# stardist/stardist

Measured on AMD Instinct MI355X. Metric: predict_instances() Mpix/s (2D) + Mvox/s (3D) end-to-end at 1/2/4/8 GPU, higher is better.
Workload: dtype f32

## Files before the change

### stardist_amd/csrc/clip_beam.h

```cpp
#pragma once
#include "clip_sweep.h"
#include <limits.h>

#if defined(BEAM_COUNT) && !defined(__HIP_DEVICE_COMPILE__)
struct BeamCounters { long beams, topx, isect_pt, isect_edges, outpt, update, maxima, lm, horz, ael_sum, il_beams, es_loads; };
inline BeamCounters& beam_counters() { static BeamCounters c = {}; return c; }
#define BEAM_CNT(f, v) (beam_counters().f += (v))
#else
#define BEAM_CNT(f, v) ((void)0)
#endif

namespace sdclip {

typedef unsigned long long u64;

enum {
  ST_OVERFLOW_AEL = 32,
  ST_OVERFLOW_LM = 64,
  ST_OVERFLOW_GJ = 128
};
enum { BEAM_MAXLM = 8 };

struct PrepPt { int x, y; };
template <bool WIDE> struct PrepIdx { typedef unsigned char type; enum { NONE = 255 }; };
template <> struct PrepIdx<true> { typedef unsigned short type; enum { NONE = 65535 }; };
template <int MAXV>
struct PolyPrep {
  typedef typename PrepIdx<(MAXV > 128)>::type pidx;
  enum { NONE = PrepIdx<(MAXV > 128)>::NONE };
  int n;
  int n_lm;
  int status;
  int pad;
  PrepPt v[MAXV + 1];
  unsigned char ecode[MAXV];
  pidx mpair[MAXV];
  pidx hlast[MAXV];
  pidx lm_left[BEAM_MAXLM], lm_right[BEAM_MAXLM];
};

#ifndef BEAM_PREP_IDX
#define BEAM_PREP_IDX short
#endif
// ... 183 lines not shown
      else if (topx(b) == topx(i) && topy(b) == topy(i) && (code[b] & 3) == 0) mp = b;
      out->mpair[i] = (typename PolyPrep<MAXV>::pidx)mp;
      int last = i, g2 = 0;
      if (is_horz(i)) {
        for (;;) {
          const int c2 = code[last] & 3;
          const int n2 = (c2 == 1) ? nx(last) : (c2 == 2 ? pv(last) : -1);
          if (n2 < 0 || !is_horz(n2)) break;
          last = n2;
          if (++g2 > MAXV) { st |= ST_ITER; break; }
        }
      }
      out->hlast[i] = (typename PolyPrep<MAXV>::pidx)last;
    }
    for (int i = 0; i < n_lm; ++i) { out->lm_left[i] = (typename PolyPrep<MAXV>::pidx)lml_[i]; out->lm_right[i] = (typename PolyPrep<MAXV>::pidx)lmr_[i]; }
    out->n = m; out->n_lm = n_lm; out->status = st;
  }
};

template <class D, class P, int MAXV, int K, int MAXIL, bool FULLGJ = false>
struct BeamCore {
  typedef PolyPrep<MAXV> Prep;
  template <bool W, int = 0> struct OrdT { typedef unsigned int type; };
  template <int D0> struct OrdT<true, D0> { typedef u64 type; };
  typedef typename OrdT<(K > 8)>::type ord_t;
  enum { ORD_BITS = (K > 8) ? 64 : 32 };
  enum { GJ = (K <= 8 ? 3 : 4), NX = (K <= 8 ? 2 : 4), EID_POLY = 4096 };
  SD_HD D& self() { return *static_cast<D*>(this); }
  static constexpr unsigned RI = P::template coord_region<K>(), RD = P::template slope_region<K>(),
                            RS = P::template region<short, K>(), RB = P::template region<signed char, K>(),
                            RIL = P::template coord_region<MAXIL>(), RILB = P::template region<signed char, MAXIL>(),
                            RG = P::template coord_region<GJ>(), RGF = P::template region<int, (FULLGJ ? GJ : 1)>(), R1 = P::template region<int, 1>(), R8 = P::template region<u64, 1>(), RO = P::template region<ord_t, 1>();
  static constexpr unsigned O_BOTX = 0, O_BOTY = O_BOTX + RI, O_TOPX = O_BOTY + RI, O_TOPY = O_TOPX + RI, O_CURX = O_TOPY + RI,
                            O_CURY = O_CURX + RI, O_DX = O_CURY + RI, O_EID = O_DX + RD, O_WCNT = O_EID + RS, O_WCNT2 = O_WCNT + RB,
                            O_OUTIDX = O_WCNT2 + RB, O_LMLC = O_OUTIDX + RB, O_WDELTA = O_LMLC + RB, O_PTYP = O_WDELTA + RB,
                            O_SIDE = O_PTYP + RB, O_ILX = O_SIDE + RB, O_ILY = O_ILX + RIL, O_ILE1 = O_ILY + RIL, O_ILE2 = O_ILE1 + RILB,
                            O_GJOP = O_ILE2 + RILB, O_GJX1 = O_GJOP + RGF, O_GJX2 = O_GJX1 + RG, O_GJY2 = O_GJX2 + RG,
                            O_XTRA = O_GJY2 + RGF, O_MLM = O_XTRA + P::template region<int, NX>(),
                            O_PA = O_MLM + P::template region<unsigned char, 16>(),
                            O_ORD = O_PA + 2 * R8, O_HSEL = O_ORD + RO, O_AFTER_ORD = O_HSEL + RO, O_PB = O_PA + R8, O_NAEL = O_AFTER_ORD, O_FREE = O_NAEL + R1, O_NLM = O_FREE + R1,
                            O_CURLM = O_NLM + R1, O_NIL = O_CURLM + R1, O_STATUS = O_NIL + R1, O_NJOINS = O_STATUS + R1,
                            O_NGJ = O_NJOINS + R1, O_NXTRA = O_NGJ + R1, O_LMY = O_NXTRA + R1, O_ORGX = O_LMY + R1, O_ORGY = O_ORGX + R1, O_CORE_END = O_ORGY + R1;
  typename P::template CoordArr<K, O_BOTX, O_ORGX, O_STATUS> botx; typename P::template CoordArr<K, O_BOTY, O_ORGY, O_STATUS> boty;
  typename P::template CoordArr<K, O_TOPX, O_ORGX, O_STATUS> topx; typename P::template CoordArr<K, O_TOPY, O_ORGY, O_STATUS> topy;
  typename P::template CoordArr<K, O_CURX, O_ORGX, O_STATUS> curx; typename P::template CoordArr<K, O_CURY, O_ORGY, O_STATUS> cury;
  typename P::template SlopeArr<K, O_DX, O_BOTX, O_BOTY, O_TOPX, O_TOPY> dx;
  typename P::template Arr<short, K, O_EID> eid;
  typename P::template Arr<signed char, K, O_WCNT> wcnt; typename P::template Arr<signed char, K, O_WCNT2> wcnt2;
  typename P::template Arr<signed char, K, O_OUTIDX> outidx;
  typename P::template Arr<signed char, K, O_LMLC> lmlc;
  typename P::template Arr<signed char, K, O_WDELTA> wdelta; typename P::template Arr<signed char, K, O_PTYP> ptyp;
  typename P::template Arr<signed char, K, O_SIDE> side;
  typename P::template CoordArr<MAXIL, O_ILX, O_ORGX, O_STATUS> ilx; typename P::template CoordArr<MAXIL, O_ILY, O_ORGY, O_STATUS> ily;
  typename P::template Arr<signed char, MAXIL, O_ILE1> ile1; typename P::template Arr<signed char, MAXIL, O_ILE2> ile2;
  typename P::template Arr<int, (FULLGJ ? GJ : 1), O_GJOP> gjop; typename P::template CoordArr<GJ, O_GJX1, O_ORGX, O_STATUS> gjx1;
  typename P::template CoordArr<GJ, O_GJX2, O_ORGX, O_STATUS> gjx2; typename P::template Arr<int, (FULLGJ ? GJ : 1), O_GJY2> gjy2;
  typename P::template Arr<int, NX, O_XTRA> xtra;
  typename P::template Arr<unsigned char, 16, O_MLM> mlm;
  typename P::template Scalar<ord_t, O_ORD> ord;
  typename P::template Scalar<ord_t, O_HSEL> hsel;
  typename P::template Scalar<const Prep*, O_PA> prepA; typename P::template Scalar<const Prep*, O_PB> prepB;
  typename P::template Scalar<int, O_NAEL> n_ael; typename P::template Scalar<int, O_FREE> freemask;
  typename P::template Scalar<int, O_NLM> n_lm; typename P::template Scalar<int, O_CURLM> cur_lm;
  typename P::template Scalar<int, O_NIL> n_il; typename P::template Scalar<int, O_STATUS> status;
  typename P::template Scalar<int, O_NJOINS> n_joins; typename P::template Scalar<int, O_NGJ> n_gj;
  typename P::template Scalar<int, O_NXTRA> n_xtra;
  typename P::template Scalar<int, O_LMY> next_lm_y;
  typename P::template Scalar<int, O_ORGX> orgx; typename P::template Scalar<int, O_ORGY> orgy;

  static constexpr ord_t ALLF = (ord_t)~(ord_t)0;
  static constexpr ord_t ONES = (ord_t)0x1111111111111111ull, HIGHS = (ord_t)0x8888888888888888ull;
  static SD_HD int nib(ord_t w, int p) { return (int)((w >> (4 * p)) & (ord_t)15); }
  static SD_HD int nib_find(ord_t w, int h) {
    const ord_t x = w ^ ((ord_t)h * ONES);
    const ord_t t = (ord_t)(x - ONES) & ~x & HIGHS;
    if (!t) return -1;
#if defined(__HIP_DEVICE_COMPILE__)
    return (ORD_BITS == 64) ? ((__ffsll((long long)t) - 1) >> 2) : ((__ffs((int)t) - 1) >> 2);
#else
    return (ORD_BITS == 64) ? (__builtin_ctzll((u64)t) >> 2) : (__builtin_ctz((unsigned)t) >> 2);
#endif
  }
  static SD_HD ord_t nib_insert(ord_t w, int p, int h) {
    const ord_t lowmask = (p == 0) ? (ord_t)0 : (ord_t)(ALLF >> (ORD_BITS - 4 * p));
    return (ord_t)((w & lowmask) | ((ord_t)h << (4 * p)) | ((ord_t)(w & ~lowmask) << 4));
  }
  static SD_HD ord_t nib_remove(ord_t w, int p) {
    const ord_t lowmask = (p == 0) ? (ord_t)0 : (ord_t)(ALLF >> (ORD_BITS - 4 * p));
    return (ord_t)((w & lowmask) | (((w >> 4) & ~lowmask)) | ((ord_t)0xF << (ORD_BITS - 4)));
  }
  static SD_HD ord_t nib_swap(ord_t w, int p, int q) {
    const ord_t d = (ord_t)(nib(w, p) ^ nib(w, q));
    return (ord_t)(w ^ (d << (4 * p)) ^ (d << (4 * q)));
  }
  SD_HD int ael_head() const { return n_ael > 0 ? nib(ord, 0) : -1; }
  SD_HD int anext(int h) const { const ord_t w = ord; const int p = nib_find(w, h); if (p < 0 || p + 1 >= n_ael) return -1; return nib(w, p + 1); }
  SD_HD int aprev(int h) const { const ord_t w = ord; const int p = nib_find(w, h); if (p <= 0) return -1; return nib(w, p - 1); }
  SD_HD bool in_ael(int h) const { return nib_find(ord, h) >= 0; }
  SD_HD int alloc_slot() {
    const int f = freemask;
    if (!f) { status |= ST_OVERFLOW_AEL; return 0; }
#if defined(__HIP_DEVICE_COMPILE__)
    const int h = __ffs(f) - 1;
#else
    const int h = __builtin_ctz((unsigned)f);
#endif
    freemask = f & (f - 1);
    return h;
  }

  SD_HD const Prep* prep_of(int id) const { return (id >= EID_POLY) ? (const Prep*)prepB : (const Prep*)prepA; }
  static SD_HD int ring_nx(const Prep* q, int i) { return i + 1 == q->n ? 0 : i + 1; }
  static SD_HD int ring_pv(const Prep* q, int i) { return i == 0 ? q->n - 1 : i - 1; }
  struct ES { int bx, by, tx, ty, code; };
  static SD_HD ES edge_static(const Prep* q, int i) {
    BEAM_CNT(es_loads, 1);
    ES s;
    s.code = q->ecode[i];
    const PrepPt p0 = q->v[i], p1 = q->v[i + 1];
    const int x0 = p0.x, y0 = p0.y, x1 = p1.x, y1 = p1.y;
    if (s.code & 4) { s.bx = x1; s.by = y1; s.tx = x0; s.ty = y0; }
    else { s.bx = x0; s.by = y0; s.tx = x1; s.ty = y1; }
    return s;
  }
  SD_HD int lml_id(int id, int code) const {
    const int c = code & 3;
    if (!c) return -1;
    const Prep* q = prep_of(id);
    const int base = id & ~(EID_POLY - 1), i = id & (EID_POLY - 1);
    return base + (c == 1 ? ring_nx(q, i) : ring_pv(q, i));
  }
  SD_HD ES es_of(int id) const { return edge_static(prep_of(id), id & (EID_POLY - 1)); }
  static SD_HD double es_dx(const ES& s) {
    const i64 dy = (i64)s.ty - s.by;
    if (dy == 0) return SD_HORIZONTAL;
    return (double)((i64)s.tx - s.bx) / (double)dy;
  }
  SD_HD void load_slot(int h, int id) {
    const ES s = es_of(id);
    botx[h] = s.bx; boty[h] = s.by; topx[h] = s.tx; topy[h] = s.ty;
    dx[h] = es_dx(s);
    eid[h] = (short)id; lmlc[h] = (signed char)(s.code & 11);
  }

  SD_HD bool is_horz(int h) const { return topy[h] == boty[h]; }
  SD_HD i64 top_x(int h, i64 y) const {
    BEAM_CNT(topx, 1);
    return (y == topy[h]) ? (i64)topx[h] : (i64)botx[h] + sd_round(dx[h] * (double)(y - boty[h]));
  }
  static SD_HD bool slopes_equal4(i64 x1, i64 y1, i64 x2, i64 y2, i64 x3, i64 y3, i64 x4, i64 y4) {
    return (y1 - y2) * (x3 - x4) == (x1 - x2) * (y3 - y4);
  }
  SD_HD bool slopes_equal_e(int e1, int e2) const {
    return ((i64)topy[e1] - boty[e1]) * ((i64)topx[e2] - botx[e2]) ==
           ((i64)topx[e1] - botx[e1]) * ((i64)topy[e2] - boty[e2]);
  }
  static SD_HD bool horz_segments_overlap(i64 a1, i64 a2, i64 b1, i64 b2) {
    if (a1 > a2) { i64 t = a1; a1 = a2; a2 = t; }
    if (b1 > b2) { i64 t = b1; b1 = b2; b2 = t; }
    return (a1 < b2) && (b1 < a2);
  }
  SD_HD void add_join(int op1, int op2, int offx, int offy) { ++n_joins; self().out_add_join(op1, op2, offx, offy); }
  SD_HD void add_ghost_join(int op, int x1, int x2, int y2) {
// ... 92 lines not shown
    int at;
    if (n == 0) at = 0;
    else if (startEdge < 0 && e2_inserts_before_e1(nib(w, 0), edge)) at = 0;
    else {
      int p = (startEdge < 0) ? 0 : nib_find(w, startEdge);
      if (p < 0) p = 0;
      while (p + 1 < n && !e2_inserts_before_e1(nib(w, p + 1), edge)) ++p;
      at = p + 1;
    }
    ord = nib_insert(w, at, edge);
    n_ael = n + 1;
  }
  SD_HD void delete_from_ael(int e) {
    const ord_t w = ord;
    const int p = nib_find(w, e);
    if (p < 0) return;
    ord = nib_remove(w, p);
    n_ael = n_ael - 1;
    freemask = freemask | (1 << e);
  }
  SD_HD void swap_positions_in_ael(int e1, int e2) {
    const ord_t w = ord;
    const int p = nib_find(w, e1), q = nib_find(w, e2);
    if (p < 0 || q < 0) return;
    ord = nib_swap(w, p, q);
  }
  SD_HD void add_edge_to_sel(int edge) { hsel = (ord_t)(((ord_t)hsel << 4) | (ord_t)edge); }
  SD_HDN int update_edge_into_ael(int e) {
    BEAM_CNT(update, 1);
    const int id = eid[e];
    const int n = lml_id(id, lmlc[e]);
    if (n < 0) { status |= ST_FAIL; return e; }
    load_slot(e, n);
    curx[e] = botx[e]; cury[e] = boty[e];
    return e;
  }

  SD_HDN void set_winding_count(int edge) {
    const ord_t w = ord;
    const int pe = nib_find(w, edge);
    int p = pe - 1;
    while (p >= 0 && (ptyp[nib(w, p)] != ptyp[edge] || wdelta[nib(w, p)] == 0)) --p;
    if (p < 0) {
      wcnt[edge] = wdelta[edge];
      wcnt2[edge] = 0;
      p = 0;
    } else {
      const int e = nib(w, p);
      if (wcnt[e] * wdelta[e] < 0) {
        int a = wcnt[e] < 0 ? -wcnt[e] : wcnt[e];
        if (a > 1) {
          if (wdelta[e] * wdelta[edge] < 0) wcnt[edge] = wcnt[e];
          else wcnt[edge] = (signed char)(wcnt[e] + wdelta[edge]);
        } else wcnt[edge] = (wdelta[edge] == 0 ? 1 : wdelta[edge]);
      } else {
        if (wdelta[edge] == 0) wcnt[edge] = (signed char)(wcnt[e] < 0 ? wcnt[e] - 1 : wcnt[e] + 1);
        else if (wdelta[e] * wdelta[edge] < 0) wcnt[edge] = wcnt[e];
        else wcnt[edge] = (signed char)(wcnt[e] + wdelta[edge]);
      }
      wcnt2[edge] = wcnt2[e];
      ++p;
    }
    for (; p < pe; ++p) wcnt2[edge] = (signed char)(wcnt2[edge] + wdelta[nib(w, p)]);
  }
  SD_HD bool is_contributing(int e) const {
    int a = wcnt[e] < 0 ? -wcnt[e] : wcnt[e];
    if (a != 1) return false;
// ... 27 lines not shown
        signed char s = side[e1]; side[e1] = side[e2]; side[e2] = s;
        signed char o = outidx[e1]; outidx[e1] = outidx[e2]; outidx[e2] = o;
      }
    } else if (c2) {
      if (e1Wc == 0 || e1Wc == 1) {
        add_out_pt_t<true>(e2, px, py);
        signed char s = side[e1]; side[e1] = side[e2]; side[e2] = s;
        signed char o = outidx[e1]; outidx[e1] = outidx[e2]; outidx[e2] = o;
      }
    } else if ((e1Wc == 0 || e1Wc == 1) && (e2Wc == 0 || e2Wc == 1)) {
      int e1Wc2 = wcnt2[e1] < 0 ? -wcnt2[e1] : wcnt2[e1];
      int e2Wc2 = wcnt2[e2] < 0 ? -wcnt2[e2] : wcnt2[e2];
      if (ptyp[e1] != ptyp[e2]) add_local_min_poly_t<true>(e1, e2, px, py);
      else if (e1Wc == 1 && e2Wc == 1) {
        if (e1Wc2 > 0 && e2Wc2 > 0) add_local_min_poly_t<true>(e1, e2, px, py);
      } else { signed char s = side[e1]; side[e1] = side[e2]; side[e2] = s; }
    }
  }

  SD_BLK void insert_local_minima_into_ael(int botY) {
    while (cur_lm < n_lm && next_lm_y == botY) {
      const int m = mlm[cur_lm];
      ++cur_lm;
      if (cur_lm < n_lm) next_lm_y = lm_y(cur_lm);
      BEAM_CNT(lm, 1);
      const int poly = (m & 128) ? 1 : 0;
      const Prep* q = poly ? (const Prep*)prepB : (const Prep*)prepA;
      const int li = q->lm_left[m & 127], ri = q->lm_right[m & 127];
      const int lb = alloc_slot();
      const int rb = alloc_slot();
      if (status & ST_OVERFLOW_AEL) return;
      load_slot(lb, poly * EID_POLY + li);
      load_slot(rb, poly * EID_POLY + ri);
      const signed char wl = (ring_nx(q, li) == ri) ? -1 : 1;
      wdelta[lb] = wl; wdelta[rb] = (signed char)-wl;
      const signed char pt = poly ? (signed char)kSubject : (signed char)kClip;
      ptyp[lb] = pt; ptyp[rb] = pt;
      curx[lb] = botx[lb]; cury[lb] = boty[lb]; side[lb] = kLeft; outidx[lb] = kUnassigned; wcnt[lb] = 0; wcnt2[lb] = 0;
      curx[rb] = botx[rb]; cury[rb] = boty[rb]; side[rb] = kRight; outidx[rb] = kUnassigned; wcnt[rb] = 0; wcnt2[rb] = 0;

      int op1 = -1; bool have_op1 = false;
      insert_edge_into_ael(lb, -1);
      insert_edge_into_ael(rb, lb);
      set_winding_count(lb);
      wcnt[rb] = wcnt[lb]; wcnt2[rb] = wcnt2[lb];
      if (is_contributing(lb)) { op1 = add_local_min_poly(lb, rb, botx[lb], boty[lb]); have_op1 = true; }
      if (is_horz(rb)) {
        add_edge_to_sel(rb);
        const int nid = lml_id(eid[rb], lmlc[rb]);
        if (nid >= 0) push_xtra(es_of(nid).ty);
      }
      if (is_horz(lb)) status |= ST_ITER;

      if (have_op1 && is_horz(rb) && n_gj > 0 && wdelta[rb] != 0) {
        const int ng = n_gj;
        for (int g = 0; g < ng; ++g)
          if (horz_segments_overlap(gjx1[g], gjx2[g], botx[rb], topx[rb])) add_join(gjop[FULLGJ ? g : 0], op1, gjx2[g], gjy2[FULLGJ ? g : 0]);
      }
      const int lp = aprev(lb);
      if (outidx[lb] >= 0 && lp >= 0 && curx[lp] == botx[lb] && outidx[lp] >= 0 &&
          slopes_equal4(botx[lp], boty[lp], topx[lp], topy[lp], curx[lb], cury[lb], topx[lb], topy[lb]) &&
          wdelta[lb] != 0 && wdelta[lp] != 0) {
        const int op2 = add_out_pt(lp, botx[lb], boty[lb]);
        add_join(op1, op2, topx[lb], topy[lb]);
      }
      if (anext(lb) != rb) {
        const int rp = aprev(rb);
        if (outidx[rb] >= 0 && rp >= 0 && outidx[rp] >= 0 &&
            slopes_equal4(curx[rp], cury[rp], topx[rp], topy[rp], curx[rb], cury[rb], topx[rb], topy[rb]) &&
            wdelta[rb] != 0 && wdelta[rp] != 0) {
          const int op2 = add_out_pt(rp, botx[rb], boty[rb]);
          add_join(op1, op2, topx[rb], topy[rb]);
        }
        int e = anext(lb);
        int guard = 0;
        while (e >= 0 && e != rb) {
          intersect_edges(rb, e, curx[lb], cury[lb]);
          e = anext(e);
          if (++guard > K) { status |= ST_ITER; break; }
        }
      }
    }
  }

  SD_HD int get_maxima_pair_id(int id) const {
    const Prep* q = prep_of(id);
    const int mp = q->mpair[id & (EID_POLY - 1)];
    return (mp == Prep::NONE) ? -1 : (id & ~(EID_POLY - 1)) + mp;
  }
  SD_HD int slot_of(int id) const {
    const ord_t w = ord; const int n = n_ael;
    for (int p = 0; p < n; ++p) { const int h = nib(w, p); if (eid[h] == id) return h; }
    return -1;
  }
  SD_HD int get_maxima_pair_ex(int e, int& slot) const {
    slot = -1;
    const int r = get_maxima_pair_id(eid[e]);
    if (r < 0) return -1;
    slot = slot_of(r);
    if (slot < 0) {
      const ES s = es_of(r);
      if (s.ty != s.by) return -1;
    }
    return r;
  }
  SD_BLK void process_horizontal(int horz) {
    BEAM_CNT(horz, 1);
    bool l2r; i64 hl, hr;
    if (botx[horz] < topx[horz]) { hl = botx[horz]; hr = topx[horz]; l2r = true; }
    else { hl = topx[horz]; hr = botx[horz]; l2r = false; }
    int eLast, eMaxPair = -1;
    {
      const int id = eid[horz];
      const Prep* q = prep_of(id);
      const int base = id & ~(EID_POLY - 1);
      const int li = q->hlast[id & (EID_POLY - 1)];
      eLast = base + li;
      if ((q->ecode[li] & 3) == 0) { const int mp = q->mpair[li]; if (mp != Prep::NONE) eMaxPair = base + mp; }
    }
    int op1 = -1; bool have_op1 = false;
    int guard = 0;
    for (;;) {
      const bool isLast = (eid[horz] == eLast);
      int e = l2r ? anext(horz) : aprev(horz);
      while (e >= 0) {
        if (++guard > 4 * K * K + 4 * MAXV) { status |= ST_ITER; return; }
        if ((l2r && curx[e] > hr) || (!l2r && curx[e] < hl)) break;
        if (curx[e] == topx[horz] && (lmlc[horz] & 3) != 0) {
          const ES s = es_of(lml_id(eid[horz], lmlc[horz]));
          if (dx[e] < es_dx(s)) break;
        }
        if (outidx[horz] >= 0) {
          op1 = add_out_pt(horz, curx[e], cury[e]);
          have_op1 = true;
          horz_joins(horz, op1);
          add_ghost_join(op1, curx[e], botx[horz], boty[horz]);
        }
        if (eid[e] == eMaxPair && isLast) {
          if (outidx[horz] >= 0) add_local_max_poly(horz, e, topx[horz], topy[horz]);
          delete_from_ael(horz);
          delete_from_ael(e);
          return;
        }
        if (l2r) intersect_edges(horz, e, curx[e], cury[horz]);
        else intersect_edges(e, horz, curx[e], cury[horz]);
        const int eNext = l2r ? anext(e) : aprev(e);
        swap_positions_in_ael(horz, e);
        e = eNext;
      }
      if ((lmlc[horz] & 8) == 0) break;
      horz = update_edge_into_ael(horz);
      if (outidx[horz] >= 0) add_out_pt(horz, botx[horz], boty[horz]);
      if (botx[horz] < topx[horz]) { hl = botx[horz]; hr = topx[horz]; l2r = true; }
      else { hl = topx[horz]; hr = botx[horz]; l2r = false; }
    }
    if (outidx[horz] >= 0 && !have_op1) {
      op1 = self().out_last_pt(horz);
      horz_joins(horz, op1);
      add_ghost_join(op1, self().out_last_pt_x(horz), topx[horz], topy[horz]);
    }
    if ((lmlc[horz] & 3) != 0) {
      if (outidx[horz] >= 0) {
        op1 = add_out_pt(horz, topx[horz], topy[horz]);
        horz = update_edge_into_ael(horz);
        if (wdelta[horz] == 0) return;
        const int ePrev = aprev(horz), eNext = anext(horz);
        if (ePrev >= 0 && curx[ePrev] == botx[horz] && cury[ePrev] == boty[horz] && wdelta[ePrev] != 0 &&
            (outidx[ePrev] >= 0 && cury[ePrev] > topy[ePrev] && slopes_equal_e(horz, ePrev))) {
          const int op2 = add_out_pt(ePrev, botx[horz], boty[horz]);
          add_join(op1, op2, topx[horz], topy[horz]);
        } else if (eNext >= 0 && curx[eNext] == botx[horz] && cury[eNext] == boty[horz] && wdelta[eNext] != 0 &&
                   outidx[eNext] >= 0 && cury[eNext] > topy[eNext] && slopes_equal_e(horz, eNext)) {
          const int op2 = add_out_pt(eNext, botx[horz], boty[horz]);
          add_join(op1, op2, topx[horz], topy[horz]);
        }
      } else update_edge_into_ael(horz);
    } else {
      if (outidx[horz] >= 0) add_out_pt(horz, topx[horz], topy[horz]);
      delete_from_ael(horz);
    }
  }
  SD_HD void process_horizontals() {
    int guard = 0;
    for (;;) {
      const ord_t w = hsel;
      const int h = (int)(w & 15u);
      if (h == 15) break;
      hsel = (ord_t)((w >> 4) | ((ord_t)0xF << (ORD_BITS - 4)));
      process_horizontal(h);
      if (++guard > 4 * MAXV) { status |= ST_ITER; break; }
    }
  }

  SD_HDN void intersect_point(int e1, int e2, i64& ipx, i64& ipy) const {
    double b1, b2;
    const double d1 = dx[e1], d2 = dx[e2];
    if (d1 == d2) { ipy = cury[e1]; ipx = top_x(e1, ipy); return; }
    else if (d1 == 0) {
      ipx = botx[e1];
      if (is_horz(e2)) ipy = boty[e2];
      else { b2 = (double)boty[e2] - ((double)botx[e2] / d2); ipy = sd_round((double)ipx / d2 + b2); }
    } else if (d2 == 0) {
      ipx = botx[e2];
      if (is_horz(e1)) ipy = boty[e1];
      else { b1 = (double)boty[e1] - ((double)botx[e1] / d1); ipy = sd_round((double)ipx / d1 + b1); }
    } else {
      b1 = (double)botx[e1] - (double)boty[e1] * d1;
      b2 = (double)botx[e2] - (double)boty[e2] * d2;
      double q = (b2 - b1) / (d1 - d2);
      ipy = sd_round(q);
      double a1 = d1 < 0 ? -d1 : d1, a2 = d2 < 0 ? -d2 : d2;
      if (a1 < a2) ipx = sd_round(d1 * q + b1);
      else ipx = sd_round(d2 * q + b2);
    }
    if (ipy < topy[e1] || ipy < topy[e2]) {
      if (topy[e1] > topy[e2]) ipy = topy[e1]; else ipy = topy[e2];
      double a1 = d1 < 0 ? -d1 : d1, a2 = d2 < 0 ? -d2 : d2;
      if (a1 < a2) ipx = top_x(e1, ipy); else ipx = top_x(e2, ipy);
    }
    if (ipy > cury[e1]) {
      ipy = cury[e1];
      double a1 = d1 < 0 ? -d1 : d1, a2 = d2 < 0 ? -d2 : d2;
      if (a1 > a2) ipx = top_x(e2, ipy); else ipx = top_x(e1, ipy);
    }
  }
  SD_BLK void build_intersect_list(int topY) {
    const int n = n_ael;
    if (n == 0) return;
    ord_t w = ord;
    for (int p = 0; p < n; ++p) { const int h = nib(w, p); curx[h] = (int)top_x(h, topY); }
    int m = n, guard = 0;
    bool isModified;
    do {
      isModified = false;
      int p = 0;
      while (p + 1 < m) {
        const int e = nib(w, p), eNext = nib(w, p + 1);
        if (curx[e] > curx[eNext]) {
          i64 px, py;
          intersect_point(e, eNext, px, py);
          if (py < topY) { px = top_x(e, topY); py = topY; }
          const int k = n_il;
          if (k < MAXIL) { ile1[k] = (signed char)e; ile2[k] = (signed char)eNext; ilx[k] = (int)px; ily[k] = (int)py; n_il = k + 1; }
          else status |= ST_OVERFLOW_IL;
          w = nib_swap(w, p, p + 1);
          isModified = true;
        }
        ++p;
        if (++guard > K * K * 2 + 8) { status |= ST_ITER; return; }
      }
      if (m > 1) --m; else break;
    } while (isModified);
  }
  SD_HDN bool fixup_intersection_order() {
    ord_t w = ord;
    const int n = n_il;
    for (int i = 1; i < n; ++i) {
      const int y = ily[i], x = ilx[i]; const signed char a = ile1[i], b = ile2[i];
      int k = i;
      while (k > 0 && ily[k - 1] < y) { ily[k] = ily[k - 1]; ilx[k] = ilx[k - 1]; ile1[k] = ile1[k - 1]; ile2[k] = ile2[k - 1]; --k; }
      if (k != i) { ily[k] = y; ilx[k] = x; ile1[k] = a; ile2[k] = b; }
    }
    for (int i = 0; i < n; ++i) {
      int p = nib_find(w, ile1[i]), q = nib_find(w, ile2[i]);
      if (!(p - q == 1 || q - p == 1)) {
        int j = i + 1;
        while (j < n) {
          const int pj = nib_find(w, ile1[j]), qj = nib_find(w, ile2[j]);
          if (pj - qj == 1 || qj - pj == 1) break;
          j++;
        }
        if (j == n) return false;
        const int y = ily[i], x = ilx[i]; const signed char a = ile1[i], b = ile2[i];
        ily[i] = ily[j]; ilx[i] = ilx[j]; ile1[i] = ile1[j]; ile2[i] = ile2[j];
        ily[j] = y; ilx[j] = x; ile1[j] = a; ile2[j] = b;
        p = nib_find(w, ile1[i]); q = nib_find(w, ile2[i]);
      }
      w = nib_swap(w, p, q);
    }
    return true;
  }
  SD_HD bool process_intersections(int topY) {
    if (n_ael == 0) return true;
    n_il = 0;
    build_intersect_list(topY);
    const int n = n_il;
    if (n == 0) return true;
    BEAM_CNT(il_beams, 1); BEAM_CNT(isect_pt, n);
    if (n == 1 || fixup_intersection_order()) {
      for (int i = 0; i < n; ++i) {
        const int e1 = ile1[i], e2 = ile2[i];
        intersect_edges(e1, e2, ilx[i], ily[i]);
        swap_positions_in_ael(e1, e2);
      }
      n_il = 0;
    } else return false;
    return true;
  }

  SD_BLK void do_maxima(int e) {
    BEAM_CNT(maxima, 1);
    int mp;
    const int mpid = get_maxima_pair_ex(e, mp);
    if (mpid < 0) {
      if (outidx[e] >= 0) add_out_pt(e, topx[e], topy[e]);
      delete_from_ael(e);
      return;
    }
    if (mp < 0) { status |= ST_FAIL; return; }
    int eNext = anext(e);
    int guard = 0;
    while (eNext >= 0 && eNext != mp) {
      intersect_edges(e, eNext, topx[e], topy[e]);
      swap_positions_in_ael(e, eNext);
      eNext = anext(e);
      if (++guard > K) { status |= ST_ITER; break; }
    }
    if (outidx[e] == kUnassigned && outidx[mp] == kUnassigned) {
      delete_from_ael(e); delete_from_ael(mp);
    } else if (outidx[e] >= 0 && outidx[mp] >= 0) {
      add_local_max_poly(e, mp, topx[e], topy[e]);
      delete_from_ael(e); delete_from_ael(mp);
    } else status |= ST_FAIL;
  }
  SD_BLK void process_edges_at_top_of_scanbeam(int topY) {
    int e = ael_head();
    int guard = 0;
    while (e >= 0) {
      if (++guard > 4 * MAXV) { status |= ST_ITER; break; }
      bool isMax = (topy[e] == topY && (lmlc[e] & 3) == 0);
      if (isMax) {
        int mps;
        const int mp = get_maxima_pair_ex(e, mps);
        bool mpHorz = false;
        if (mp >= 0) { if (mps >= 0) mpHorz = is_horz(mps); else mpHorz = true; }
        isMax = (mp < 0 || !mpHorz);
      }
      if (isMax) {
        const int ePrev = aprev(e);
        do_maxima(e);
        if (status & ST_FAIL) return;
        e = (ePrev < 0) ? ael_head() : anext(ePrev);
      } else {
        if (topy[e] == topY && (lmlc[e] & 8) != 0) {
          e = update_edge_into_ael(e);
          if (outidx[e] >= 0) add_out_pt(e, botx[e], boty[e]);
          add_edge_to_sel(e);
        } else {
          curx[e] = (int)top_x(e, topY);
          cury[e] = topY;
        }
        e = anext(e);
      }
    }
    process_horizontals();
    e = ael_head();
    guard = 0;
    while (e >= 0) {
      if (++guard > 4 * MAXV) { status |= ST_ITER; break; }
      if (topy[e] == topY && (lmlc[e] & 3) != 0) {
        bool op = false; int oph = -1;
        if (outidx[e] >= 0) { oph = add_out_pt(e, topx[e], topy[e]); op = true; }
        e = update_edge_into_ael(e);
        const int ePrev = aprev(e), eNext = anext(e);
        if (ePrev >= 0 && curx[ePrev] == botx[e] && cury[ePrev] == boty[e] && op &&
            outidx[ePrev] >= 0 && cury[ePrev] > topy[ePrev] &&
            slopes_equal4(curx[e], cury[e], topx[e], topy[e], curx[ePrev], cury[ePrev], topx[ePrev], topy[ePrev]) &&
            wdelta[e] != 0 && wdelta[ePrev] != 0) {
          const int op2 = add_out_pt(ePrev, botx[e], boty[e]);
          add_join(oph, op2, topx[e], topy[e]);
        } else if (eNext >= 0 && curx[eNext] == botx[e] && cury[eNext] == boty[e] && op &&
                   outidx[eNext] >= 0 && cury[eNext] > topy[eNext] &&
                   slopes_equal4(curx[e], cury[e], topx[e], topy[e], curx[eNext], cury[eNext], topx[eNext], topy[eNext]) &&
                   wdelta[e] != 0 && wdelta[eNext] != 0) {
          const int op2 = add_out_pt(eNext, botx[e], boty[e]);
          add_join(oph, op2, topx[e], topy[e]);
        }
      }
      e = anext(e);
    }
  }

  SD_HD void reset_core(const Prep* a, const Prep* b) {
    prepA = a; prepB = b;
    orgx = a->n ? a->v[0].x : (b->n ? b->v[0].x : 0); orgy = a->n ? a->v[0].y : (b->n ? b->v[0].y : 0);
    ord = ALLF; hsel = ALLF; n_ael = 0; freemask = (1 << K) - 1;
    n_lm = 0; cur_lm = 0; n_il = 0; status = ST_OK; n_joins = 0; n_gj = 0; n_xtra = 0;
  }
  SD_BLK bool run_sweep() {
    const Prep* a = prepA; const Prep* b = prepB;
    status |= (a->status | b->status);
    {
      const int na = a->n ? a->n_lm : 0, nb = b->n ? b->n_lm : 0;
      if (na + nb > 16) { status |= ST_OVERFLOW_LM; return false; }
      int ia = 0, ib = 0, k = 0;
      while (ia < na || ib < nb) {
        bool takeA;
        if (ia >= na) takeA = false;
        else if (ib >= nb) takeA = true;
        else takeA = edge_static(a, a->lm_left[ia]).by >= edge_static(b, b->lm_left[ib]).by;
        if (takeA) { mlm[k] = (unsigned char)ia; ++ia; } else { mlm[k] = (unsigned char)(128 + ib); ++ib; }
        ++k;
      }
      n_lm = k;
    }
    if (n_lm == 0) return true;
    cur_lm = 0;
    next_lm_y = lm_y(0);
    int botY = next_lm_y, topY = 0;
    int guard = 0;
    bool ok = true;
    for (;;) {
      insert_local_minima_into_ael(botY);
      if (status & (ST_OVERFLOW_AEL | ST_OVERFLOW_REC | ST_OVERFLOW_IL | ST_ITER)) { ok = false; break; }
      const bool popped = pop_scanbeam(botY, topY);
      if (!popped) break;
      if (++guard > 4 * MAXV + 8) { status |= ST_ITER; break; }
      BEAM_CNT(beams, 1); BEAM_CNT(ael_sum, n_ael);
      process_horizontals();
      n_gj = 0;
      if (!process_intersections(topY)) { ok = false; break; }
      process_edges_at_top_of_scanbeam(topY);
      if (status & ST_FAIL) { ok = false; break; }
      botY = topY;
    }
    if (!ok || (status & ST_FAIL)) { status |= ST_FAIL; return false; }
    return true;
  }
};

template <int MAXV, int K, int MAXIL, int MAXREC, class P = PlainStorage>
struct Beam : BeamCore<Beam<MAXV, K, MAXIL, MAXREC, P>, P, MAXV, K, MAXIL> {
  typedef BeamCore<Beam<MAXV, K, MAXIL, MAXREC, P>, P, MAXV, K, MAXIL> B;
  using B::outidx; using B::side; using B::status; using B::ord; using B::n_ael;
  static constexpr unsigned RR = P::template coord_region<MAXREC>();
  static constexpr unsigned O_RFX = B::O_CORE_END, O_RFY = O_RFX + RR, O_RLX = O_RFY + RR, O_RLY = O_RLX + RR, O_RSUM = O_RLY + RR,
                            O_RSER = O_RSUM + P::template region<i64, MAXREC>(), O_NREC = O_RSER + P::template region<unsigned char, MAXREC>(),
                            O_RFREE = O_NREC + P::template region<int, 1>(), O_TWICE = O_RFREE + P::template region<int, 1>(),
                            O_SABS = O_TWICE + P::template region<i64, 1>(), O_END = O_SABS + P::template region<i64, 1>();
  typename P::template CoordArr<MAXREC, O_RFX, B::O_ORGX, B::O_STATUS> rfx; typename P::template CoordArr<MAXREC, O_RFY, B::O_ORGY, B::O_STATUS> rfy;
  typename P::template CoordArr<MAXREC, O_RLX, B::O_ORGX, B::O_STATUS> rlx; typename P::template CoordArr<MAXREC, O_RLY, B::O_ORGY, B::O_STATUS> rly;
  typename P::template Arr<i64, MAXREC, O_RSUM> rsum;
  static constexpr unsigned lds_bytes() { return O_END; }
  typename P::template Arr<unsigned char, MAXREC, O_RSER> rser;
  typename P::template Scalar<int, O_NREC> n_rec;
  typename P::template Scalar<int, O_RFREE> rfree;
  typename P::template Scalar<i64, O_TWICE> twice_area;
  typename P::template Scalar<i64, O_SABS> sum_abs_terms;
  SD_HD void term(i64 c) { sum_abs_terms += sd_abs64(c); }
  SD_HDN int out_add_pt(int e, int px, int py) { return out_add_pt_i(e, px, py); }
  SD_HDN void out_append(int e1, int e2) { out_append_i(e1, e2); }
  SD_HD int out_add_pt_i(int e, int px, int py) {
    int r = outidx[e];
    if (r < 0) {
      const int f = rfree;
// ... 78 lines not shown
```

### stardist_amd/csrc/clip_sweep.h

```cpp
#pragma once
#include <stdint.h>

#if defined(__HIPCC__)
#define SD_HD __host__ __device__ __forceinline__
#if defined(SD_SWEEP_INLINE)
#define SD_HDN __host__ __device__ __forceinline__
#else
#define SD_HDN __host__ __device__ __noinline__
#endif
#else
#define SD_HD inline
#define SD_HDN inline
#endif
#if defined(SD_BEAM_BLOCKS_AS_CALLS)
#define SD_BLK SD_HDN
#else
#define SD_BLK SD_HD
#endif

namespace sdclip {

typedef long long i64;

enum { kUnassigned = -1 };
enum { kLeft = 1, kRight = 2 };
enum { kClip = 1, kSubject = 0 };
enum {
  ST_OK = 0,
  ST_OVERFLOW_IL = 1,
  ST_OVERFLOW_REC = 2,
  ST_SORT_DEPTH = 4,
  ST_FAIL = 8,
  ST_ITER = 16
};

#define SD_HORIZONTAL (-1.0E+40)

SD_HD i64 sd_round(double v) { return (v < 0) ? (i64)(v - 0.5) : (i64)(v + 0.5); }
SD_HD i64 sd_cross(int ax, int ay, int bx, int by) { return (i64)ax * by - (i64)ay * bx; }
SD_HD i64 sd_abs64(i64 v) { return v < 0 ? -v : v; }

template <typename T>
struct StdSort {
  static SD_HD bool comp(const T& a, const T& b) { return b.y < a.y; }
  static SD_HD void swp(T& a, T& b) { T t = a; a = b; b = t; }
  static SD_HD void unguarded_linear_insert(T* a, int last) {
    T val = a[last];
    int next = last - 1;
    while (comp(val, a[next])) { a[last] = a[next]; last = next; --next; }
    a[last] = val;
// ... 812 lines not shown
      intersect_edges(e, eNext, topx[e], topy[e]);
      swap_positions_in_ael(e, eNext);
      eNext = anext[e];
      if (++guard > NE) { status |= ST_ITER; break; }
    }
    if (outidx[e] == kUnassigned && outidx[eMaxPair] == kUnassigned) {
      delete_from_ael(e); delete_from_ael(eMaxPair);
    } else if (outidx[e] >= 0 && outidx[eMaxPair] >= 0) {
      add_local_max_poly(e, eMaxPair, topx[e], topy[e]);
      delete_from_ael(e); delete_from_ael(eMaxPair);
    } else status |= ST_FAIL;
  }
  SD_BLK void process_edges_at_top_of_scanbeam(int topY) {
    int e = ael;
    int guard = 0;
    while (e >= 0) {
      if (++guard > 4 * NE) { status |= ST_ITER; break; }
      bool isMax = (topy[e] == topY && lml[e] < 0);
      if (isMax) {
        int mp = get_maxima_pair_ex(e);
        isMax = (mp < 0 || !is_horz(mp));
      }
      if (isMax) {
        int ePrev = aprev[e];
        do_maxima(e);
        if (status & ST_FAIL) return;
        e = (ePrev < 0) ? (int)ael : (int)anext[ePrev];
      } else {
        if (topy[e] == topY && lml[e] >= 0 && is_horz(lml[e])) {
          e = update_edge_into_ael(e);
          if (outidx[e] >= 0) add_out_pt(e, botx[e], boty[e]);
          add_edge_to_sel(e);
        } else {
          curx[e] = (int)top_x(e, topY);
          cury[e] = topY;
        }
        e = anext[e];
      }
    }
    process_horizontals();
    e = ael;
    guard = 0;
    while (e >= 0) {
      if (++guard > 4 * NE) { status |= ST_ITER; break; }
      if (topy[e] == topY && lml[e] >= 0) {
        bool op = false; int oph = -1;
        if (outidx[e] >= 0) { oph = add_out_pt(e, topx[e], topy[e]); op = true; }
        e = update_edge_into_ael(e);
        int ePrev = aprev[e], eNext = anext[e];
        if (ePrev >= 0 && curx[ePrev] == botx[e] && cury[ePrev] == boty[e] && op &&
            outidx[ePrev] >= 0 && cury[ePrev] > topy[ePrev] &&
            slopes_equal4(curx[e], cury[e], topx[e], topy[e], curx[ePrev], cury[ePrev], topx[ePrev], topy[ePrev]) &&
            wdelta[e] != 0 && wdelta[ePrev] != 0) {
          const int op2 = add_out_pt(ePrev, botx[e], boty[e]);
          add_join(oph, op2, topx[e], topy[e]);
        } else if (eNext >= 0 && curx[eNext] == botx[e] && cury[eNext] == boty[e] && op &&
                   outidx[eNext] >= 0 && cury[eNext] > topy[eNext] &&
                   slopes_equal4(curx[e], cury[e], topx[e], topy[e], curx[eNext], cury[eNext], topx[eNext], topy[eNext]) &&
                   wdelta[e] != 0 && wdelta[eNext] != 0) {
          const int op2 = add_out_pt(eNext, botx[e], boty[e]);
          add_join(oph, op2, topx[e], topy[e]);
        }
      }
      e = anext[e];
    }
  }

// ... 115 lines not shown
```

Measured before the change: 333.1.

## Replace per-edge cury with scanline scalar and drop redundant curx recomputation

```diff
diff --git a/stardist_amd/csrc/clip_beam.h b/stardist_amd/csrc/clip_beam.h
--- a/stardist_amd/csrc/clip_beam.h
+++ b/stardist_amd/csrc/clip_beam.h
@@ -9,6 +9,11 @@
 #else
 #define BEAM_CNT(f, v) ((void)0)
 #endif
+#ifndef BEAM_PH
+#define BEAM_PH(i) ((void)0)
+#endif
+enum { BEAM_PH_PREP = 0, BEAM_PH_SETUP, BEAM_PH_LM, BEAM_PH_POP, BEAM_PH_HORZ, BEAM_PH_ILIST, BEAM_PH_ISECT, BEAM_PH_TOP_EDGES, BEAM_PH_TOP_HORZ,
+       BEAM_PH_TOP_UPDATE, BEAM_PH_END, BEAM_PH_COUNT };
 
 namespace sdclip {
 
@@ -258,7 +263,7 @@
                             RIL = P::template coord_region<MAXIL>(), RILB = P::template region<signed char, MAXIL>(),
                             RG = P::template coord_region<GJ>(), RGF = P::template region<int, (FULLGJ ? GJ : 1)>(), R1 = P::template region<int, 1>(), R8 = P::template region<u64, 1>(), RO = P::template region<ord_t, 1>();
   static constexpr unsigned O_BOTX = 0, O_BOTY = O_BOTX + RI, O_TOPX = O_BOTY + RI, O_TOPY = O_TOPX + RI, O_CURX = O_TOPY + RI,
-                            O_CURY = O_CURX + RI, O_DX = O_CURY + RI, O_EID = O_DX + RD, O_WCNT = O_EID + RS, O_WCNT2 = O_WCNT + RB,
+                            O_DX = O_CURX + RI, O_EID = O_DX + RD, O_WCNT = O_EID + RS, O_WCNT2 = O_WCNT + RB,
                             O_OUTIDX = O_WCNT2 + RB, O_LMLC = O_OUTIDX + RB, O_WDELTA = O_LMLC + RB, O_PTYP = O_WDELTA + RB,
                             O_SIDE = O_PTYP + RB, O_ILX = O_SIDE + RB, O_ILY = O_ILX + RIL, O_ILE1 = O_ILY + RIL, O_ILE2 = O_ILE1 + RILB,
                             O_GJOP = O_ILE2 + RILB, O_GJX1 = O_GJOP + RGF, O_GJX2 = O_GJX1 + RG, O_GJY2 = O_GJX2 + RG,
@@ -266,10 +271,11 @@
                             O_PA = O_MLM + P::template region<unsigned char, 16>(),
                             O_ORD = O_PA + 2 * R8, O_HSEL = O_ORD + RO, O_AFTER_ORD = O_HSEL + RO, O_PB = O_PA + R8, O_NAEL = O_AFTER_ORD, O_FREE = O_NAEL + R1, O_NLM = O_FREE + R1,
                             O_CURLM = O_NLM + R1, O_NIL = O_CURLM + R1, O_STATUS = O_NIL + R1, O_NJOINS = O_STATUS + R1,
-                            O_NGJ = O_NJOINS + R1, O_NXTRA = O_NGJ + R1, O_LMY = O_NXTRA + R1, O_ORGX = O_LMY + R1, O_ORGY = O_ORGX + R1, O_CORE_END = O_ORGY + R1;
+                            O_NGJ = O_NJOINS + R1, O_NXTRA = O_NGJ + R1, O_LMY = O_NXTRA + R1, O_ORGX = O_LMY + R1, O_ORGY = O_ORGX + R1, O_SCANY = O_ORGY + R1, O_RINGN = O_SCANY + R1,
+                            O_CORE_END = O_RINGN + P::template region<int, 2>();
   typename P::template CoordArr<K, O_BOTX, O_ORGX, O_STATUS> botx; typename P::template CoordArr<K, O_BOTY, O_ORGY, O_STATUS> boty;
   typename P::template CoordArr<K, O_TOPX, O_ORGX, O_STATUS> topx; typename P::template CoordArr<K, O_TOPY, O_ORGY, O_STATUS> topy;
-  typename P::template CoordArr<K, O_CURX, O_ORGX, O_STATUS> curx; typename P::template CoordArr<K, O_CURY, O_ORGY, O_STATUS> cury;
+  typename P::template CoordArr<K, O_CURX, O_ORGX, O_STATUS> curx;
   typename P::template SlopeArr<K, O_DX, O_BOTX, O_BOTY, O_TOPX, O_TOPY> dx;
   typename P::template Arr<short, K, O_EID> eid;
   typename P::template Arr<signed char, K, O_WCNT> wcnt; typename P::template Arr<signed char, K, O_WCNT2> wcnt2;
@@ -293,6 +299,8 @@
   typename P::template Scalar<int, O_NXTRA> n_xtra;
   typename P::template Scalar<int, O_LMY> next_lm_y;
   typename P::template Scalar<int, O_ORGX> orgx; typename P::template Scalar<int, O_ORGY> orgy;
+  typename P::template Scalar<int, O_SCANY> scan_y;
+  typename P::template Arr<int, 2, O_RINGN> ring_n;
 
   static constexpr ord_t ALLF = (ord_t)~(ord_t)0;
   static constexpr ord_t ONES = (ord_t)0x1111111111111111ull, HIGHS = (ord_t)0x8888888888888888ull;
@@ -336,8 +344,8 @@
   }
 
   SD_HD const Prep* prep_of(int id) const { return (id >= EID_POLY) ? (const Prep*)prepB : (const Prep*)prepA; }
-  static SD_HD int ring_nx(const Prep* q, int i) { return i + 1 == q->n ? 0 : i + 1; }
-  static SD_HD int ring_pv(const Prep* q, int i) { return i == 0 ? q->n - 1 : i - 1; }
+  static SD_HD int ring_nx(int n, int i) { return i + 1 == n ? 0 : i + 1; }
+  static SD_HD int ring_pv(int n, int i) { return i == 0 ? n - 1 : i - 1; }
   struct ES { int bx, by, tx, ty, code; };
   static SD_HD ES edge_static(const Prep* q, int i) {
     BEAM_CNT(es_loads, 1);
@@ -352,9 +360,9 @@
   SD_HD int lml_id(int id, int code) const {
     const int c = code & 3;
     if (!c) return -1;
-    const Prep* q = prep_of(id);
+    const int n = ring_n[id >= EID_POLY ? 1 : 0];
     const int base = id & ~(EID_POLY - 1), i = id & (EID_POLY - 1);
-    return base + (c == 1 ? ring_nx(q, i) : ring_pv(q, i));
+    return base + (c == 1 ? ring_nx(n, i) : ring_pv(n, i));
   }
   SD_HD ES es_of(int id) const { return edge_static(prep_of(id), id & (EID_POLY - 1)); }
   static SD_HD double es_dx(const ES& s) {
@@ -513,7 +521,7 @@
     const int n = lml_id(id, lmlc[e]);
     if (n < 0) { status |= ST_FAIL; return e; }
     load_slot(e, n);
-    curx[e] = botx[e]; cury[e] = boty[e];
+    curx[e] = botx[e];
     return e;
   }
 
@@ -607,12 +615,12 @@
       if (status & ST_OVERFLOW_AEL) return;
       load_slot(lb, poly * EID_POLY + li);
       load_slot(rb, poly * EID_POLY + ri);
-      const signed char wl = (ring_nx(q, li) == ri) ? -1 : 1;
+      const signed char wl = (ring_nx(ring_n[poly], li) == ri) ? -1 : 1;
       wdelta[lb] = wl; wdelta[rb] = (signed char)-wl;
       const signed char pt = poly ? (signed char)kSubject : (signed char)kClip;
       ptyp[lb] = pt; ptyp[rb] = pt;
-      curx[lb] = botx[lb]; cury[lb] = boty[lb]; side[lb] = kLeft; outidx[lb] = kUnassigned; wcnt[lb] = 0; wcnt2[lb] = 0;
-      curx[rb] = botx[rb]; cury[rb] = boty[rb]; side[rb] = kRight; outidx[rb] = kUnassigned; wcnt[rb] = 0; wcnt2[rb] = 0;
+      curx[lb] = botx[lb]; side[lb] = kLeft; outidx[lb] = kUnassigned; wcnt[lb] = 0; wcnt2[lb] = 0;
+      curx[rb] = botx[rb]; side[rb] = kRight; outidx[rb] = kUnassigned; wcnt[rb] = 0; wcnt2[rb] = 0;
 
       int op1 = -1; bool have_op1 = false;
       insert_edge_into_ael(lb, -1);
@@ -634,7 +642,7 @@
       }
       const int lp = aprev(lb);
       if (outidx[lb] >= 0 && lp >= 0 && curx[lp] == botx[lb] && outidx[lp] >= 0 &&
-          slopes_equal4(botx[lp], boty[lp], topx[lp], topy[lp], curx[lb], cury[lb], topx[lb], topy[lb]) &&
+          slopes_equal4(botx[lp], boty[lp], topx[lp], topy[lp], curx[lb], scan_y, topx[lb], topy[lb]) &&
           wdelta[lb] != 0 && wdelta[lp] != 0) {
         const int op2 = add_out_pt(lp, botx[lb], boty[lb]);
         add_join(op1, op2, topx[lb], topy[lb]);
@@ -642,7 +650,7 @@
       if (anext(lb) != rb) {
         const int rp = aprev(rb);
         if (outidx[rb] >= 0 && rp >= 0 && outidx[rp] >= 0 &&
-            slopes_equal4(curx[rp], cury[rp], topx[rp], topy[rp], curx[rb], cury[rb], topx[rb], topy[rb]) &&
+            slopes_equal4(curx[rp], scan_y, topx[rp], topy[rp], curx[rb], scan_y, topx[rb], topy[rb]) &&
             wdelta[rb] != 0 && wdelta[rp] != 0) {
           const int op2 = add_out_pt(rp, botx[rb], boty[rb]);
           add_join(op1, op2, topx[rb], topy[rb]);
@@ -650,7 +658,7 @@
         int e = anext(lb);
         int guard = 0;
         while (e >= 0 && e != rb) {
-          intersect_edges(rb, e, curx[lb], cury[lb]);
+          intersect_edges(rb, e, curx[lb], scan_y);
           e = anext(e);
           if (++guard > K) { status |= ST_ITER; break; }
         }
@@ -706,7 +714,7 @@
           if (dx[e] < es_dx(s)) break;
         }
         if (outidx[horz] >= 0) {
-          op1 = add_out_pt(horz, curx[e], cury[e]);
+          op1 = add_out_pt(horz, curx[e], scan_y);
           have_op1 = true;
           horz_joins(horz, op1);
           add_ghost_join(op1, curx[e], botx[horz], boty[horz]);
@@ -717,8 +725,8 @@
           delete_from_ael(e);
           return;
         }
-        if (l2r) intersect_edges(horz, e, curx[e], cury[horz]);
-        else intersect_edges(e, horz, curx[e], cury[horz]);
+        if (l2r) intersect_edges(horz, e, curx[e], scan_y);
+        else intersect_edges(e, horz, curx[e], scan_y);
         const int eNext = l2r ? anext(e) : aprev(e);
         swap_positions_in_ael(horz, e);
         e = eNext;
@@ -740,12 +748,12 @@
         horz = update_edge_into_ael(horz);
         if (wdelta[horz] == 0) return;
         const int ePrev = aprev(horz), eNext = anext(horz);
-        if (ePrev >= 0 && curx[ePrev] == botx[horz] && cury[ePrev] == boty[horz] && wdelta[ePrev] != 0 &&
-            (outidx[ePrev] >= 0 && cury[ePrev] > topy[ePrev] && slopes_equal_e(horz, ePrev))) {
+        if (ePrev >= 0 && curx[ePrev] == botx[horz] && scan_y == boty[horz] && wdelta[ePrev] != 0 &&
+            (outidx[ePrev] >= 0 && scan_y > topy[ePrev] && slopes_equal_e(horz, ePrev))) {
           const int op2 = add_out_pt(ePrev, botx[horz], boty[horz]);
           add_join(op1, op2, topx[horz], topy[horz]);
-        } else if (eNext >= 0 && curx[eNext] == botx[horz] && cury[eNext] == boty[horz] && wdelta[eNext] != 0 &&
-                   outidx[eNext] >= 0 && cury[eNext] > topy[eNext] && slopes_equal_e(horz, eNext)) {
+        } else if (eNext >= 0 && curx[eNext] == botx[horz] && scan_y == boty[horz] && wdelta[eNext] != 0 &&
+                   outidx[eNext] >= 0 && scan_y > topy[eNext] && slopes_equal_e(horz, eNext)) {
           const int op2 = add_out_pt(eNext, botx[horz], boty[horz]);
           add_join(op1, op2, topx[horz], topy[horz]);
         }
@@ -770,7 +778,7 @@
   SD_HDN void intersect_point(int e1, int e2, i64& ipx, i64& ipy) const {
     double b1, b2;
     const double d1 = dx[e1], d2 = dx[e2];
-    if (d1 == d2) { ipy = cury[e1]; ipx = top_x(e1, ipy); return; }
+    if (d1 == d2) { ipy = scan_y; ipx = top_x(e1, ipy); return; }
     else if (d1 == 0) {
       ipx = botx[e1];
       if (is_horz(e2)) ipy = boty[e2];
@@ -793,8 +801,8 @@
       double a1 = d1 < 0 ? -d1 : d1, a2 = d2 < 0 ? -d2 : d2;
       if (a1 < a2) ipx = top_x(e1, ipy); else ipx = top_x(e2, ipy);
     }
-    if (ipy > cury[e1]) {
-      ipy = cury[e1];
+    if (ipy > scan_y) {
+      ipy = scan_y;
       double a1 = d1 < 0 ? -d1 : d1, a2 = d2 < 0 ? -d2 : d2;
       if (a1 > a2) ipx = top_x(e2, ipy); else ipx = top_x(e1, ipy);
     }
@@ -859,6 +867,7 @@
     if (n_ael == 0) return true;
     n_il = 0;
     build_intersect_list(topY);
+    BEAM_PH(BEAM_PH_ILIST);
     const int n = n_il;
     if (n == 0) return true;
     BEAM_CNT(il_beams, 1); BEAM_CNT(isect_pt, n);
@@ -899,9 +908,11 @@
     } else status |= ST_FAIL;
   }
   SD_BLK void process_edges_at_top_of_scanbeam(int topY) {
-    int e = ael_head();
+    ord_t w = ord;
+    int n = n_ael, p = 0;
     int guard = 0;
-    while (e >= 0) {
+    while (p < n) {
+      int e = nib(w, p);
       if (++guard > 4 * MAXV) { status |= ST_ITER; break; }
       bool isMax = (topy[e] == topY && (lmlc[e] & 3) == 0);
       if (isMax) {
@@ -912,52 +923,53 @@
         isMax = (mp < 0 || !mpHorz);
       }
       if (isMax) {
-        const int ePrev = aprev(e);
         do_maxima(e);
         if (status & ST_FAIL) return;
-        e = (ePrev < 0) ? ael_head() : anext(ePrev);
+        w = ord; n = n_ael;
       } else {
         if (topy[e] == topY && (lmlc[e] & 8) != 0) {
           e = update_edge_into_ael(e);
           if (outidx[e] >= 0) add_out_pt(e, botx[e], boty[e]);
           add_edge_to_sel(e);
         } else {
-          curx[e] = (int)top_x(e, topY);
-          cury[e] = topY;
+#if defined(BEAM_VERIFY_CURX) && !defined(__HIP_DEVICE_COMPILE__)
+          { const int stored = curx[e]; curx[e] = (int)top_x(e, topY); sd_curx_checks()[0] += 1; sd_curx_checks()[1] += (stored != (int)curx[e]); }
+#endif
         }
-        e = anext(e);
-      }
-    }
+        ++p;
+      }
+    }
+    scan_y = topY;
+    BEAM_PH(BEAM_PH_TOP_EDGES);
     process_horizontals();
-    e = ael_head();
-    guard = 0;
-    while (e >= 0) {
-      if (++guard > 4 * MAXV) { status |= ST_ITER; break; }
+    BEAM_PH(BEAM_PH_TOP_HORZ);
+    w = ord; n = n_ael;
+    for (p = 0; p < n; ++p) {
+      int e = nib(w, p);
       if (topy[e] == topY && (lmlc[e] & 3) != 0) {
         bool op = false; int oph = -1;
         if (outidx[e] >= 0) { oph = add_out_pt(e, topx[e], topy[e]); op = true; }
         e = update_edge_into_ael(e);
-        const int ePrev = aprev(e), eNext = anext(e);
-        if (ePrev >= 0 && curx[ePrev] == botx[e] && cury[ePrev] == boty[e] && op &&
-            outidx[ePrev] >= 0 && cury[ePrev] > topy[ePrev] &&
-            slopes_equal4(curx[e], cury[e], topx[e], topy[e], curx[ePrev], cury[ePrev], topx[ePrev], topy[ePrev]) &&
+        const int ePrev = p > 0 ? nib(w, p - 1) : -1, eNext = p + 1 < n ? nib(w, p + 1) : -1;
+        if (ePrev >= 0 && curx[ePrev] == botx[e] && scan_y == boty[e] && op &&
+            outidx[ePrev] >= 0 && scan_y > topy[ePrev] &&
+            slopes_equal4(curx[e], scan_y, topx[e], topy[e], curx[ePrev], scan_y, topx[ePrev], topy[ePrev]) &&
             wdelta[e] != 0 && wdelta[ePrev] != 0) {
           const int op2 = add_out_pt(ePrev, botx[e], boty[e]);
           add_join(oph, op2, topx[e], topy[e]);
-        } else if (eNext >= 0 && curx[eNext] == botx[e] && cury[eNext] == boty[e] && op &&
-                   outidx[eNext] >= 0 && cury[eNext] > topy[eNext] &&
-                   slopes_equal4(curx[e], cury[e], topx[e], topy[e], curx[eNext], cury[eNext], topx[eNext], topy[eNext]) &&
+        } else if (eNext >= 0 && curx[eNext] == botx[e] && scan_y == boty[e] && op &&
+                   outidx[eNext] >= 0 && scan_y > topy[eNext] &&
+                   slopes_equal4(curx[e], scan_y, topx[e], topy[e], curx[eNext], scan_y, topx[eNext], topy[eNext]) &&
                    wdelta[e] != 0 && wdelta[eNext] != 0) {
           const int op2 = add_out_pt(eNext, botx[e], boty[e]);
           add_join(oph, op2, topx[e], topy[e]);
         }
       }
-      e = anext(e);
     }
   }
 
   SD_HD void reset_core(const Prep* a, const Prep* b) {
-    prepA = a; prepB = b;
+    prepA = a; prepB = b; ring_n[0] = a->n; ring_n[1] = b->n;
     orgx = a->n ? a->v[0].x : (b->n ? b->v[0].x : 0); orgy = a->n ? a->v[0].y : (b->n ? b->v[0].y : 0);
     ord = ALLF; hsel = ALLF; n_ael = 0; freemask = (1 << K) - 1;
     n_lm = 0; cur_lm = 0; n_il = 0; status = ST_OK; n_joins = 0; n_gj = 0; n_xtra = 0;
@@ -983,19 +995,27 @@
     cur_lm = 0;
     next_lm_y = lm_y(0);
     int botY = next_lm_y, topY = 0;
+    scan_y = botY;
+    BEAM_PH(BEAM_PH_SETUP);
     int guard = 0;
     bool ok = true;
     for (;;) {
       insert_local_minima_into_ael(botY);
+      BEAM_PH(BEAM_PH_LM);
       if (status & (ST_OVERFLOW_AEL | ST_OVERFLOW_REC | ST_OVERFLOW_IL | ST_ITER)) { ok = false; break; }
       const bool popped = pop_scanbeam(botY, topY);
+      BEAM_PH(BEAM_PH_POP);
       if (!popped) break;
       if (++guard > 4 * MAXV + 8) { status |= ST_ITER; break; }
       BEAM_CNT(beams, 1); BEAM_CNT(ael_sum, n_ael);
       process_horizontals();
+      BEAM_PH(BEAM_PH_HORZ);
       n_gj = 0;
-      if (!process_intersections(topY)) { ok = false; break; }
+      const bool isect_ok = process_intersections(topY);
+      BEAM_PH(BEAM_PH_ISECT);
+      if (!isect_ok) { ok = false; break; }
       process_edges_at_top_of_scanbeam(topY);
+      BEAM_PH(BEAM_PH_TOP_UPDATE);
       if (status & ST_FAIL) { ok = false; break; }
       botY = topY;
     }
diff --git a/stardist_amd/csrc/clip_sweep.h b/stardist_amd/csrc/clip_sweep.h
--- a/stardist_amd/csrc/clip_sweep.h
+++ b/stardist_amd/csrc/clip_sweep.h
@@ -16,6 +16,10 @@
 #define SD_BLK SD_HDN
 #else
 #define SD_BLK SD_HD
+#endif
+
+#if defined(BEAM_VERIFY_CURX) && !defined(__HIP_DEVICE_COMPILE__)
+inline long* sd_curx_checks() { static long c[2] = {0, 0}; return c; }
 #endif
 
 namespace sdclip {
@@ -894,7 +898,9 @@
           if (outidx[e] >= 0) add_out_pt(e, botx[e], boty[e]);
           add_edge_to_sel(e);
         } else {
-          curx[e] = (int)top_x(e, topY);
+#if defined(BEAM_VERIFY_CURX) && !defined(__HIP_DEVICE_COMPILE__)
+          { const int stored = curx[e]; curx[e] = (int)top_x(e, topY); sd_curx_checks()[0] += 1; sd_curx_checks()[1] += (stored != (int)curx[e]); }
+#endif
           cury[e] = topY;
         }
         e = anext[e];
```

Measured after the change: 341.0 (median of 6 runs). +2.4%, better.
